# Berkeley-Speech-Group/sylber

Hardware: AMD Instinct MI355X
Metric: audio-sec/s encoded (sylber_base, 16 kHz, batched 10 s clips) (higher is better)
Workload: dtype bf16

## Files before the change

### include/sylber_hip_dev.h

```cpp
#ifndef SYLBER_HIP_DEV_H
#define SYLBER_HIP_DEV_H
#include <stdint.h>
#include "sylber_hip.h"
#ifdef __cplusplus
extern "C" {
#endif
int sylber_debug_gemm_bench(int32_t M, int32_t N, int32_t K, int32_t ldx, int32_t epi, int32_t act, int32_t cfg,
                            int32_t iters, float* ms_out);
int sylber_debug_gemm_pick(int32_t M, int32_t N, int32_t K, int32_t epi, int32_t act, int32_t fmt, int32_t model, int32_t kpat);
int sylber_debug_gemm_trace(int32_t M, int32_t N, int32_t K, int32_t ldx, int32_t epi, int32_t act, unsigned long long* out20,
                            float* ms_out);
int sylber_debug_poison_workspace(sylber_t h, int32_t byte);
int sylber_debug_conv0_scale_shift(sylber_t h, int32_t B, float* out_host);
int sylber_debug_attention_bench(int32_t B, int32_t T, int32_t precision, int32_t iters, float* ms_out);
#ifdef __cplusplus
}
#endif
#endif
```

### sylber_amd/_lib.py

```python
from __future__ import annotations

import ctypes
import os
from ctypes import POINTER, c_char_p, c_float, c_int, c_int32, c_int64, c_void_p

_HERE = os.path.dirname(os.path.abspath(__file__))
LIB_PATH = os.path.join(_HERE, "libsylber_hip.so")
_DEV_LIB = False
MAX_LAYERS = 12

c_float_p = POINTER(c_float)


class SylberLayerWeights(ctypes.Structure):
    _fields_ = [(n, c_float_p) for n in (
        "q_w", "q_b", "k_w", "k_b", "v_w", "v_b", "o_w", "o_b", "ln1_w", "ln1_b",
        "ff1_w", "ff1_b", "ff2_w", "ff2_b", "ln2_w", "ln2_b")]


class SylberMlpHidden(ctypes.Structure):
    _fields_ = [(n, c_float_p) for n in ("lin_w", "lin_b", "ff1_w", "ff1_b", "ff2_w", "ff2_b", "ln_w", "ln_b")]


class SylberMlpWeights(ctypes.Structure):
# ... 154 lines not shown
    "sylber_forward_packed": (c_int, [c_void_p, c_void_p, POINTER(c_int32), c_int32, c_void_p, c_void_p]),
    "sylber_packed_gather": (c_int, [c_void_p, POINTER(c_int32), c_int32, c_void_p, c_void_p]),
    "sylber_segment_packed": (c_int, [c_void_p, c_void_p, POINTER(c_int32), c_int32, c_float, c_float, c_void_p, c_void_p, c_void_p,
                                      c_void_p]),
    "sylber_cfm_packed_layout": (c_int, [POINTER(c_int32), c_int32, POINTER(c_int32)]),
    "sylber_cfm_workspace_bytes_packed": (c_int64, [c_void_p, POINTER(c_int32), c_int32]),
    "sylber_cfm_sample_packed": (c_int, [c_void_p, c_void_p, POINTER(c_int32), c_int32, c_int32, c_void_p, c_float, c_void_p, c_void_p,
                                         c_void_p]),
    "sylber_condition_packed_workspace_floats": (c_int64, [c_void_p, c_int32, c_int32]),
    "sylber_condition_packed": (c_int, [c_void_p, c_void_p, POINTER(c_int32), POINTER(c_int32), c_int32, c_void_p, c_void_p, c_void_p,
                                        c_int32, c_int32, c_float, c_void_p, c_void_p, c_void_p, c_void_p]),
    "sylber_condition_units_packed": (c_int, [c_void_p, c_void_p, c_int32, c_void_p, c_int32, c_void_p, c_void_p, c_void_p,
                                              POINTER(c_int32), c_int32, c_int32, c_void_p, c_void_p, c_void_p]),
    "sylber_op_attention": (c_int, [c_void_p, c_void_p, c_void_p, c_void_p, c_void_p, c_int32, c_int32, c_int32,
                                    c_int32, c_void_p]),
}
DEV_EXPORTS = {
    "sylber_debug_gemm_bench": (c_int, [c_int32] * 8 + [POINTER(c_float)]),
    "sylber_debug_gemm_pick": (c_int, [c_int32] * 8),
    "sylber_debug_gemm_trace": (c_int, [c_int32] * 6 + [POINTER(ctypes.c_uint64), POINTER(c_float)]),
    "sylber_debug_attention_bench": (c_int, [c_int32] * 4 + [POINTER(c_float)]),
    "sylber_debug_poison_workspace": (c_int, [c_void_p, c_int32]),
    "sylber_debug_conv0_scale_shift": (c_int, [c_void_p, c_int32, c_void_p]),
}
OPT_GEMM_TILE, OPT_ATTN_QUERIES_PER_WAVE, OPT_GEMM_PERSISTENT = 1, 2, 3
OPT_FUSE_OUTPROJ_LN, OPT_CONV0_VALU = 4, 5
OPT_FP8_ATTENTION, OPT_SEGMENT, OPT_PER_UTTERANCE = 7, 9, 14
TAP_CONV0, TAP_PROJ, TAP_POSCONV = -1, -2, -3
LTAP_QKV, LTAP_CTX, LTAP_ATTN_SUM, LTAP_LN1, LTAP_FFN1, LTAP_FFN2_SUM = 0, 1, 2, 3, 4, 5
LTAP_WIDTH = {LTAP_QKV: 2304, LTAP_CTX: 768, LTAP_ATTN_SUM: 768, LTAP_LN1: 768, LTAP_FFN1: 3072, LTAP_FFN2_SUM: 768}


def TAP_LAYER(l: int, k: int) -> int:
    return -(8 * (int(l) + 1) + int(k))


_LIB = None


class SylberHipError(RuntimeError):
    pass


def load() -> ctypes.CDLL:
    global _LIB
    if _LIB is None:
# ... 26 lines not shown
```

### sylber_amd/csrc/api.hip

```cpp
#include "ctx.h"

static thread_local char g_err[512] = "";
void syl_set_error(const char* what, const char* detail) { snprintf(g_err, sizeof(g_err), "%s: %s", what, detail); }
extern "C" const char* sylber_last_error(void) { return g_err; }

struct Packer {
    std::vector<char> host;
    size_t add(size_t bytes) { size_t off = (host.size() + 255) & ~(size_t)255; host.resize(off + bytes); return off; }
    size_t add_f32(const float* src, size_t n) { size_t o = add(n * 4); memcpy(host.data() + o, src, n * 4); return o; }
    int fmt = FMT_BF16;
    size_t add_bf16(const float* src, size_t n) {
        if (fmt == FMT_SPLIT) {
            size_t o = add(n * 4);
            bf16_t* d = (bf16_t*)(host.data() + o);
            for (size_t i = 0; i < n; ++i) { d[i] = f2h_host(src[i]); d[n + i] = f2h_host(src[i] - h2f_host(d[i])); }
            return o;
        }
        size_t o = add(n * 2);
        bf16_t* d = (bf16_t*)(host.data() + o);
        if (fmt == FMT_F16) for (size_t i = 0; i < n; ++i) d[i] = f2h_host(src[i]);
        else for (size_t i = 0; i < n; ++i) d[i] = f2bf(src[i]);
        return o;
    }
};
// ... 14 lines not shown
    size_t o_gnw = P.add_f32(w->gn_w, 512), o_gnb = P.add_f32(w->gn_b, 512);
    size_t o_conv[7] = {0};
    for (int i = 1; i < 7; ++i) {
        const int k = CK[i];
        const bool chunk_major = k == 3 && !f32 && c->fmt_conv != FMT_SPLIT;
        std::vector<float> tmp((size_t)512 * k * 512);
        for (int o = 0; o < 512; ++o)
            for (int cc = 0; cc < 512; ++cc)
                for (int j = 0; j < k; ++j) tmp[((size_t)o * k + j) * 512 + cc] = w->conv_w[i][((size_t)o * 512 + cc) * k + j];
        if (chunk_major) {
            std::vector<float> t2(tmp.size());
            for (int o = 0; o < 512; ++o)
                for (int pos = 0; pos < 1536; ++pos)
                    t2[(size_t)o * 1536 + pos] = tmp[(size_t)o * 1536 + tap3_offset(pos * 2) / 2];
            tmp.swap(t2);
        }
        o_conv[i] = f32 ? P.add_f32(tmp.data(), tmp.size()) : P.add_bf16(tmp.data(), tmp.size());
    }
    P.fmt = c->fmt;
    size_t o_fplw = P.add_f32(w->fp_ln_w, 512), o_fplb = P.add_f32(w->fp_ln_b, 512);
    size_t o_fpw = f32 ? P.add_f32(w->fp_w, 768 * 512) : P.add_bf16(w->fp_w, 768 * 512), o_fpb = P.add_f32(w->fp_b, 768);
    size_t o_posw;
    {
        std::vector<float> tmp((size_t)16 * 128 * 64 * 56, 0.f);
        for (int g = 0; g < 16; ++g)
            for (int n = 0; n < 48; ++n)
                for (int cc = 0; cc < 48; ++cc)
                    for (int t = 0; t < 128; ++t)
                        tmp[(((size_t)g * 128 + t) * 64 + n) * 56 + cc] = w->pos_w[(((size_t)g * 48 + n) * 48 + cc) * 128 + t];
        if (!f32) o_posw = P.add_bf16(tmp.data(), tmp.size());
        else {
            std::vector<float> t32((size_t)16 * 128 * 64 * 52, 0.f);
            for (int g = 0; g < 16; ++g)
                for (int n = 0; n < 48; ++n)
                    for (int cc = 0; cc < 48; ++cc)
                        for (int t = 0; t < 128; ++t)
                            t32[(((size_t)g * 128 + t) * 64 + n) * 52 + cc] = w->pos_w[(((size_t)g * 48 + n) * 48 + cc) * 128 + t];
            o_posw = P.add_f32(t32.data(), t32.size());
        }
    }
    size_t o_posb = P.add_f32(w->pos_b, 768);
    size_t o_elw = P.add_f32(w->enc_ln_w, 768), o_elb = P.add_f32(w->enc_ln_b, 768);
    struct LOff { size_t wqkv, bqkv, wo, bo, l1w, l1b, w1, b1, w2, b2, l2w, l2b; } lo[SYLBER_MAX_LAYERS];
    for (int l = 0; l < w->num_layers; ++l) {
        const SylberLayerWeights& lw = w->layers[l];
        std::vector<float> qkv((size_t)2304 * 768), bq(2304);
        memcpy(qkv.data(), lw.q_w, 768 * 768 * 4);
        memcpy(qkv.data() + 768 * 768, lw.k_w, 768 * 768 * 4);
        memcpy(qkv.data() + 2 * 768 * 768, lw.v_w, 768 * 768 * 4);
        memcpy(bq.data(), lw.q_b, 768 * 4); memcpy(bq.data() + 768, lw.k_b, 768 * 4); memcpy(bq.data() + 1536, lw.v_b, 768 * 4);
        lo[l].wqkv = f32 ? P.add_f32(qkv.data(), qkv.size()) : P.add_bf16(qkv.data(), qkv.size()); lo[l].bqkv = P.add_f32(bq.data(), 2304);
        lo[l].wo = f32 ? P.add_f32(lw.o_w, 768 * 768) : P.add_bf16(lw.o_w, 768 * 768); lo[l].bo = P.add_f32(lw.o_b, 768);
        lo[l].l1w = P.add_f32(lw.ln1_w, 768); lo[l].l1b = P.add_f32(lw.ln1_b, 768);
        lo[l].w1 = f32 ? P.add_f32(lw.ff1_w, (size_t)3072 * 768) : P.add_bf16(lw.ff1_w, (size_t)3072 * 768); lo[l].b1 = P.add_f32(lw.ff1_b, 3072);
// ... 232 lines not shown
```

### sylber_amd/csrc/common.h

```cpp
#pragma once
#include <hip/hip_runtime.h>
#include <stdint.h>

typedef unsigned short bf16_t;
typedef __bf16 bf16x8_t __attribute__((ext_vector_type(8)));
typedef float f32x16_t __attribute__((ext_vector_type(16)));
typedef float f32x4_t __attribute__((ext_vector_type(4)));
typedef unsigned short u16x8_t __attribute__((ext_vector_type(8)));
typedef unsigned short u16x4_t __attribute__((ext_vector_type(4)));

#define SYL_HIDDEN 768
#define SYL_CONV 512
#define SYL_SLOT_SAMPLES 320
#define SYL_HEADS 12
#define SYL_HDIM 64
#define SYL_FFN 3072
#define SYL_POSK 128
#define SYL_POSG 16
#define SYL_POSC 48

__host__ __device__ __forceinline__ bf16_t f2bf(float f) {
    union { float f; uint32_t u; } v; v.f = f;
    uint32_t u = v.u;
    if ((u & 0x7fffffffu) > 0x7f800000u) return (bf16_t)((u >> 16) | 0x40);
    u += 0x7fffu + ((u >> 16) & 1u);
    return (bf16_t)(u >> 16);
}
__host__ __device__ __forceinline__ float bf2f(bf16_t h) {
    union { float f; uint32_t u; } v; v.u = ((uint32_t)h) << 16;
    return v.f;
}
typedef __bf16 bf16x2_t __attribute__((ext_vector_type(2)));
__device__ __forceinline__ uint32_t pack_bf16x2(float lo, float hi) {
    typedef float f32pair_t __attribute__((ext_vector_type(2)));
    const f32pair_t v = {lo, hi};
    return __builtin_bit_cast(uint32_t, __builtin_convertvector(v, bf16x2_t));
}
__device__ __forceinline__ bf16_t f2bf_dev(float f) { return __builtin_bit_cast(unsigned short, (__bf16)f); }

enum { FMT_BF16 = 0, FMT_F16 = 1, FMT_SPLIT = 2 };
typedef _Float16 f16x8_t __attribute__((ext_vector_type(8)));
typedef _Float16 f16x2_t __attribute__((ext_vector_type(2)));
#define SYL_Q_SCALE 0.18033688011112042f
template <int FMT> struct H16 {
    static __device__ __forceinline__ uint32_t pack2(float lo, float hi) { return pack_bf16x2(lo, hi); }
    static __device__ __forceinline__ uint32_t pack2_bounded(float lo, float hi) { return pack_bf16x2(lo, hi); }
    static __device__ __forceinline__ bf16_t cvt(float f) { return f2bf_dev(f); }
    static __device__ __forceinline__ float up(bf16_t h) { return bf2f(h); }
    static __device__ __forceinline__ f32x16_t mfma(bf16x8_t a, bf16x8_t b, f32x16_t c) {
        return __builtin_amdgcn_mfma_f32_32x32x16_bf16(a, b, c, 0, 0, 0);
    }
};
template <> struct H16<FMT_F16> {
    static __device__ __forceinline__ float sat(float f) { return __builtin_amdgcn_fmed3f(f, -65504.0f, 65504.0f); }
    static __device__ __forceinline__ uint32_t pack2(float lo, float hi) {
        typedef float f32pair_t __attribute__((ext_vector_type(2)));
        const f32pair_t v = {sat(lo), sat(hi)};
        return __builtin_bit_cast(uint32_t, __builtin_convertvector(v, f16x2_t));
    }
    static __device__ __forceinline__ uint32_t pack2_bounded(float lo, float hi) {
        typedef float f32pair_t __attribute__((ext_vector_type(2)));
        const f32pair_t v = {lo, hi};
        return __builtin_bit_cast(uint32_t, __builtin_convertvector(v, f16x2_t));
    }
    static __device__ __forceinline__ bf16_t cvt(float f) { return __builtin_bit_cast(unsigned short, (_Float16)sat(f)); }
    static __device__ __forceinline__ float up(bf16_t h) { return (float)__builtin_bit_cast(_Float16, h); }
    static __device__ __forceinline__ f32x16_t mfma(bf16x8_t a, bf16x8_t b, f32x16_t c) {
        return __builtin_amdgcn_mfma_f32_32x32x16_f16(__builtin_bit_cast(f16x8_t, a), __builtin_bit_cast(f16x8_t, b), c, 0, 0, 0);
    }
};
template <> struct H16<FMT_SPLIT> : H16<FMT_F16> {
    static __device__ __forceinline__ uint32_t pack2_lo(float lo, float hi, uint32_t hi2) {
        const f16x2_t h = __builtin_bit_cast(f16x2_t, hi2);
        return H16<FMT_F16>::pack2_bounded(lo - (float)h[0], hi - (float)h[1]);
    }
    static __device__ __forceinline__ bf16_t cvt_lo(float f, bf16_t hi) { return H16<FMT_F16>::cvt(f - H16<FMT_F16>::up(hi)); }
};
__host__ __forceinline__ bf16_t f2h_host(float f) {
    union { float f; uint32_t u; } v; v.f = f;
    const uint32_t sign = (v.u >> 16) & 0x8000u;
    uint32_t a = v.u & 0x7fffffffu;
    if (a > 0x7f800000u) return (bf16_t)(sign | 0x7e00u);
    if (a >= 0x477ff000u) return (bf16_t)(sign | 0x7bffu);
    if (a < 0x38800000u) {
        if (a < 0x33000000u) return (bf16_t)sign;
        const int e = (int)(a >> 23);
        const uint32_t m = (a & 0x7fffffu) | 0x800000u;
        const int shift = 126 - e;
        uint32_t r = m >> shift;
        const uint32_t rem = m & ((1u << shift) - 1u), half = 1u << (shift - 1);
        if (rem > half || (rem == half && (r & 1u))) ++r;
// ... 133 lines not shown
```

### sylber_amd/csrc/forward.hip

```cpp
#include "ctx.h"

extern "C" int32_t sylber_num_frames(int32_t n) {
    for (int i = 0; i < 7; ++i) n = (n - CK[i]) / CS[i] + 1;
    return n;
}

static int frames_needed(int Lmax) {
    int n = Lmax, tp = 0;
    for (int i = 0; i < 7; ++i) {
        n = (n - CK[i]) / CS[i] + 1;
        const int f = 1 << (6 - i);
        const int need = (n + f - 1) / f;
        tp = need > tp ? need : tp;
    }
    return tp;
}
static int padded_frames(int Lmax) { return (frames_needed(Lmax) + 31) & ~31; }
extern "C" int32_t sylber_padded_frames(int32_t n_samples) { return n_samples < 400 ? 0 : padded_frames(n_samples); }

#define SYL_SLOT_ALIGN 64
extern "C" int sylber_packed_layout(const int32_t* samples_host, int32_t B, int32_t* offsets, int32_t* frames) {
    if (!samples_host || !offsets || !frames || B < 1) { syl_set_error("sylber_packed_layout", "need B >= 1 and non-null arrays"); return 1; }
    const long long cap = (long long)INT32_MAX / SYL_SLOT_SAMPLES;
    long long off = 0;
// ... 315 lines not shown
        return g;
    }
    void residual(GemmArgs& g, const float* gamma, const float* beta) const {
        g.out0 = w.pre; g.ld0 = 768; g.res = w.pre; g.ldres = 768; g.ln_stats = w.stats; g.ln_gamma = gamma; g.ln_beta = beta;
    }

    int projection() {
        LnArgs a = {};
        a.in = feats; a.in_bf16 = 1; a.ld_in = 512; a.gamma = c->fp_ln_w; a.beta = c->fp_ln_b;
        a.out_bf16 = w.ln512; a.ld_bf16 = 512; a.M = M; a.D = 512; a.fmt = c->fmt; a.fmt_in = c->fmt_conv;
        a.in_lo = feats_lo; a.out_lo = p.lo_ln512;
        RUN("ln512", launch_layernorm(a, s));
        GemmArgs g = linear(w.ln512, p.lo_ln512, c->fp_w, c->fp_b, 768, 512);
        g.out0 = w.xf32; g.ld0 = 768; g.out1 = w.xpad; g.Tp = p.Tp; g.T = p.T; g.valid = w.valid; g.xpad_rows = p.Tp + 128; g.out_lo = p.lo_xpad;
        RUN("gemm_proj", launch_gemm_bf16(EPI_PROJ, g, s));
        if (pk) RUN("zero_slot_tails", launch_zero_slot_tails(w.xf32, w.xpad, pk->slot, pk->frames, pk->nclip, pk->tail_max, s));
        AUDIT(aud_e, AUD_LN512, w.ln512, M, 512, 512);
        AUDIT(aud_e, AUD_XPAD, w.xpad, (long)B * (p.Tp + 128), 768, 768);
        return 0;
    }

    int posconv() {
        if (pk) RUN("posconv", launch_posconv_packed(w.xpad, c->pos_w, c->pos_b, w.xf32, w.pre, pk->nclip, pk->slot_max, pk->slot, pk->frames, s, c->fmt));
        else RUN("posconv", launch_posconv(w.xpad, c->pos_w, c->pos_b, w.xf32, w.pre, B, p.Tp, split ? 2 : 1, s, c->fmt, p.lo_xpad, (long)16 * 128 * 64 * 56));
        return 0;
    }

    int layernorm(const float* gam, const float* bet, bool last) {
        LnArgs a = {};
        a.in = w.pre; a.in_bf16 = 0; a.ld_in = 768; a.gamma = gam; a.beta = bet; a.M = M; a.D = 768; a.fmt = c->fmt; a.fmt_in = c->fmt;
        if (last) { a.out_f32 = hidden_dev; a.ld_f32 = 768; a.Tp = p.Tp; a.T = p.T; }
        else if (f8) { a.out_fp8 = w8.h; a.ld_fp8 = 768; a.out_scale = w8.hs; a.scale_rows = w8.Mp; a.out_stats = w.stats; }
        else { a.out_bf16 = w.h; a.ld_bf16 = 768; a.out_stats = w.stats; a.out_lo = p.lo_hbf; }
        if (launch_layernorm(a, s)) return 1;
        AUDIT(aud_e && !last && !f8, AUD_LN, w.h, M, 768, 768);
        return 0;
    }

    int tap_rows16(const bf16_t* buf, long lo, int W) {
        tapped = true;
        RUN("copy_out", launch_bf16_to_f32_rows(buf, W, hidden_dev, B, p.Tp, p.T, W, s, c->fmt, lo));
        return 0;
    }
    int tap_pre() { tapped = true; return copy_frames_f32(w.pre, hidden_dev, B, p.Tp, p.T, s); }

    int layer16(const LayerDev& d, bool last, int tk) {
        GemmArgs g = linear(w.h, p.lo_hbf, d.wqkv, d.bqkv, 2304, 768);
// ... 333 lines not shown
```

### sylber_amd/csrc/frontend.hip

```cpp
#include <stdlib.h>

#include "kernels.h"

#define NSTAT 65
#define C0_ROWS 256

__global__ __launch_bounds__(256) void conv0_stats_kernel(const float* __restrict__ wav, int Lmax, int L0, int chunk,
                                                          double* __restrict__ partials, int nchunk, const int* __restrict__ rows,
                                                          const int* __restrict__ slot) {
    const int b = blockIdx.y, ck = blockIdx.x;
    const float* x = wav + (slot ? (size_t)SYL_SLOT_SAMPLES * slot[b] : (size_t)b * Lmax);
    if (rows) {
        L0 = rows[b];
        const int nck = (L0 + 2047) / 2048;
        chunk = (L0 + nck - 1) / nck;
    }
    const int l0 = ck * chunk;
    const int l1 = min(L0, l0 + chunk);
    double acc[NSTAT];
#pragma unroll
    for (int i = 0; i < NSTAT; ++i) acc[i] = 0.0;
    for (int l = l0 + threadIdx.x; l < l1; l += 256) {
        float v[10];
#pragma unroll
// ... 181 lines not shown
    const int l_blk = bx * C0_ROWS;
    __syncthreads();
    for (int i = tid; i < C0_ROWS * 5 + 16; i += 256) {
        const int idx = 5 * l_blk + i;
        xs[i] = idx < Lmax ? x[idx] : 0.f;
    }
    __syncthreads();
#pragma unroll 1
    for (int rb = 0; rb < 2; ++rb) {
        const int lrow0 = wave * 64 + rb * 32;
        const int l0 = l_blk + lrow0;
        if (l0 >= R0) break;
        f16x8_t xh, xl;
        {
            const float* xr = xs + 5 * (lrow0 + ml) + 8 * h;
#pragma unroll
            for (int j = 0; j < 8; ++j) {
                const float v = xr[j];
                const _Float16 vh = (_Float16)v;
                xh[j] = vh; xl[j] = (_Float16)(v - (float)vh);
            }
        }
        const bool live = l0 + ml < L0;
#pragma unroll 1
        for (int q4 = 0; q4 < 4; ++q4) {
#pragma unroll
            for (int bi = 0; bi < 4; ++bi) {
                const int blk = q4 * 4 + bi;
                const f16x8_t whi = *(const f16x8_t*)(wfr + (blk * 64 + lane) * 32);
                const f16x8_t wlo = *(const f16x8_t*)(wfr + (blk * 64 + lane) * 32 + 16);
                f32x16_t acc;
#pragma unroll
                for (int g = 0; g < 4; ++g) {
                    const float4 sv = *(const float4*)(shf + 32 * blk + 8 * g + 4 * h);
                    acc[4 * g + 0] = sv.x; acc[4 * g + 1] = sv.y; acc[4 * g + 2] = sv.z; acc[4 * g + 3] = sv.w;
                }
                acc = __builtin_amdgcn_mfma_f32_32x32x16_f16(whi, xh, acc, 0, 0, 0);
                acc = __builtin_amdgcn_mfma_f32_32x32x16_f16(whi, xl, acc, 0, 0, 0);
                acc = __builtin_amdgcn_mfma_f32_32x32x16_f16(wlo, xh, acc, 0, 0, 0);
#pragma unroll
                for (int g = 0; g < 4; ++g) {
                    float y0 = gelu_fast(acc[4 * g + 0]), y1 = gelu_fast(acc[4 * g + 1]), y2 = gelu_fast(acc[4 * g + 2]), y3 = gelu_fast(acc[4 * g + 3]);
                    if (!live) { y0 = y1 = y2 = y3 = 0.f; }
                    uint2 pk; pk.x = H16<FMT>::pack2(y0, y1); pk.y = H16<FMT>::pack2(y2, y3);
                    *(uint2*)(stg + ml * (256 + 16) + (32 * bi + 8 * g + 4 * h) * 2) = pk;
                }
            }
#pragma unroll
            for (int it = 0; it < 8; ++it) {
                const int idx = it * 64 + lane;
                const int r = idx >> 4, ch = idx & 15;
                typedef unsigned int u32x4_t __attribute__((ext_vector_type(4)));
                const u32x4_t v = *(const u32x4_t*)(stg + r * (256 + 16) + ch * 16);
                const int l = l0 + r;
                if constexpr (NOSTORE) { if (v.x == 0x7fc1dead && l < 0) out[0] = (bf16_t)v.y; }
                else if (l < R0) __builtin_nontemporal_store(v, (u32x4_t*)(out + (obase + l) * SYL_CONV + q4 * 128 + ch * 8));
            }
        }
    }
    }
}

int launch_conv0_stats(const float* wav, int B, int Lmax, int L0, double* partials, int nchunk, hipStream_t s, const int* rows, const int* slot) {
    const int chunk = (L0 + nchunk - 1) / nchunk;
    hipLaunchKernelGGL(conv0_stats_kernel, dim3(nchunk, B), dim3(256), 0, s, wav, Lmax, L0, chunk, partials, nchunk, rows, slot);
    HIP_TRY(hipGetLastError());
    return 0;
}
int launch_conv0_finalize(const double* partials, int nchunk, const float* w0, const float* gn_w, const float* gn_b, int B,
                          int L0, float* scale_shift, hipStream_t s, const int* rows) {
    hipLaunchKernelGGL(conv0_finalize_kernel, dim3(B), dim3(512), 0, s, partials, nchunk, w0, gn_w, gn_b, L0, scale_shift, rows);
    HIP_TRY(hipGetLastError());
    return 0;
}
int launch_conv0_gn_gelu(const float* wav, int B, int Lmax, int L0, int R0, const float* w0, const float* scale_shift,
                         void* out, int out_f32, hipStream_t s, int fmt, long out_lo, int valu16) {
    dim3 grid((R0 + C0_ROWS - 1) / C0_ROWS, B);
    if (out_f32)
        hipLaunchKernelGGL((conv0_gn_gelu_kernel<true, true, FMT_BF16>), grid, dim3(256), 0, s, wav, Lmax, L0, R0, w0, scale_shift, out, 0L);
    else if (fmt == FMT_SPLIT)
        hipLaunchKernelGGL((conv0_gn_gelu_kernel<false, true, FMT_SPLIT>), grid, dim3(256), 0, s, wav, Lmax, L0, R0, w0, scale_shift, out, out_lo);
// ... 230 lines not shown
```

### sylber_amd/csrc/kernels.h

```cpp
#pragma once
#include "common.h"

enum GemmAct { ACT_NONE = 0, ACT_GELU_FAST = 1, ACT_GELU_ERF = 2, ACT_GELU_ERF7 = 3 };
enum GemmEpi {
    EPI_BF16 = 0,
    EPI_F32 = 1,
    EPI_F32_RES = 2,
    EPI_QK = 3,
    EPI_PROJ = 4,
    EPI_MXFP8 = 7,
    EPI_QK8 = 8,
    EPI_F32_RESLN = 6,
};

struct GemmArgs {
    const bf16_t* X; long ldx;
    const bf16_t* W;
    int M, N, K;
    int M_store;
    const float* bias;
    int act;
    void* out0; long ld0;
    void* out1; void* out2;
    const float* res; long ldres;
// ... 82 lines not shown
    const float* gamma; const float* beta;
    float* out_f32; long ld_f32;
    bf16_t* out_bf16; long ld_bf16;
    uint8_t* out_fp8; long ld_fp8;
    uint8_t* out_scale; long scale_rows;
    float* out_stats;
    int M, D;
    int Tp, T;
    long in_lo, out_lo;
};
int launch_layernorm(const LnArgs& a, hipStream_t s);

int launch_attention(const bf16_t* q, const bf16_t* k, const bf16_t* vt, const int* valid, bf16_t* ctx, int B, int T,
                     int Tp, int Tpv, int qw, hipStream_t s, int fmt = 0, long lo_qk = 0, long lo_vt = 0, long lo_ctx = 0);
int launch_attention_f8(const uint8_t* q8, const uint8_t* qs, const uint8_t* k8, const uint8_t* ks, const uint8_t* v8, const uint8_t* vs,
                        const int* valid, void* ctx, uint8_t* ctx_scale, long scale_rows, int B, int T, int Tp, int Tpv, hipStream_t s);
int launch_attention_f8out(const bf16_t* q, const bf16_t* k, const bf16_t* vt, const int* valid, uint8_t* ctx8, uint8_t* ctx_scale,
                           long scale_rows, int B, int T, int Tp, int Tpv, int qw, hipStream_t s);
int launch_attention_f32(const float* q, const float* k, const float* v, const int* valid, float* ctx, int B, int T,
                         int Tp, hipStream_t s);

int launch_posconv(const bf16_t* xpad, const bf16_t* wpk, const float* bias, const float* x_f32, float* out, int B,
                   int Tp, int act, hipStream_t s, int fmt = 0, long x_lo = 0, long w_lo = 0);
int launch_posconv_f32(const float* xpad, const float* w, const float* bias, const float* x_f32, float* out, int B,
                       int Tp, hipStream_t s);

int launch_segment(const float* hidden, int B, int T, int D, float norm_thr, float merge_thr, int64_t* seg, int* nseg,
                   float* feat, float* scratch, hipStream_t s, int mode = 0, const int* frames = nullptr, const int* row0 = nullptr);
size_t segment_scratch_floats(int B, int T, int D);

int launch_upload_ints(int* dst, const int32_t* vals_host, int n, int add, hipStream_t s);
int launch_f32_to_bf16(const float* in, bf16_t* out, size_t n, hipStream_t s);
int launch_f32_to_split16(const float* in, bf16_t* out, long lo_off, size_t n, hipStream_t s);
int launch_bf16_to_f32_rows(const bf16_t* in, long ld_in, float* out, int B, int Tp, int T, int D, hipStream_t s, int fmt = 0, long in_lo = 0);
int launch_tap_qkv(const bf16_t* q, const bf16_t* k, const bf16_t* vt, float* out, int B, int T, int Tp, int Tpv, hipStream_t s, int fmt, long lo_qk, long lo_vt);
```

### sylber_amd/csrc/ops.hip

```cpp
#include "ctx.h"

struct TmpBuf {
    void* p = nullptr;
    ~TmpBuf() { if (p) hipFree(p); }
    int alloc(size_t bytes) { return hipMalloc(&p, bytes) == hipSuccess ? 0 : 1; }
};

static void decode_tile(int tile, GemmArgs& g) {
    if (tile >= 1000000) { g.tune_mfma16 = -1; tile -= 1000000; if (tile == 999) tile = -1; }
    const int t = tile >= 100000 ? tile / 100000 : 0;
    if (tile >= 100000) tile %= 100000;
    g.tune_tail = t == 0 ? 0 : (t == 1 ? -1 : t - 1);
    g.tune_cfg = tile < 0 ? 0 : tile % 1000 + 1;
    g.tune_persist = tile >= 9000 ? -1 : (tile >= 1000 ? tile / 1000 : 0);
}

extern "C" int sylber_op_linear(const float* a_dev, const float* w_dev, const float* bias_dev, float* c_dev, int32_t M,
                                int32_t N, int32_t K, int32_t act, int32_t precision, int32_t tile, void* stream) {
    hipStream_t s = (hipStream_t)stream;
    if (precision == SYLBER_FP8) {
        if (K % 128 != 0) { syl_set_error("sylber_op_linear", "fp8 needs K % 128 == 0"); return 1; }
        TmpBuf a8, as, w8, wsc;
        const long Mp = ((long)M + 255) & ~255L, Np = ((long)N + 255) & ~255L;
        if (a8.alloc((size_t)M * K) || as.alloc((size_t)Mp * (K / 32)) || w8.alloc((size_t)N * K) || wsc.alloc((size_t)Np * (K / 32))) {
// ... 228 lines not shown
    const int qw = queries_per_wave == 32 ? 1 : (queries_per_wave == 64 ? 2 : 0);
    TmpBuf qb, kb, vb, cb;
    const size_t n = (size_t)B * Tp * 768;
    if (qb.alloc(n * 2) || kb.alloc(n * 2 + 64 * 64 * 2) || vb.alloc((size_t)B * 768 * Tpv * 2) || cb.alloc(n * 2)) { syl_set_error("sylber_op_attention", "alloc"); return 1; }
    HIP_TRY(hipMemsetAsync(qb.p, 0, n * 2, s)); HIP_TRY(hipMemsetAsync(kb.p, 0, n * 2 + 64 * 64 * 2, s));
    HIP_TRY(hipMemsetAsync(vb.p, 0, (size_t)B * 768 * Tpv * 2, s)); HIP_TRY(hipMemsetAsync(cb.p, 0, n * 2, s));
    hipLaunchKernelGGL(pack_qkv_kernel, dim3(T, B), dim3(256), 0, s, q_dev, k_dev, v_dev, (bf16_t*)qb.p, (bf16_t*)kb.p, (bf16_t*)vb.p, T, Tp, Tpv);
    if (launch_attention((bf16_t*)qb.p, (bf16_t*)kb.p, (bf16_t*)vb.p, valid_dev, (bf16_t*)cb.p, B, T, Tp, Tpv, qw, s)) return 1;
    if (launch_bf16_to_f32_rows((bf16_t*)cb.p, 768, o_dev, B, Tp, T, 768, s)) return 1;
    HIP_TRY(hipStreamSynchronize(s));
    return 0;
}


__global__ void fill_random_bf16(bf16_t* p, size_t n, unsigned seed);
extern "C" int sylber_debug_poison_workspace(sylber_t c, int32_t byte) {
    if (!c) { syl_set_error("sylber_debug_poison_workspace", "null handle"); return 1; }
    GUARD_DEVICE(c->device);
    HIP_TRY(hipDeviceSynchronize());
    if (c->ws) HIP_TRY(hipMemset(c->ws, byte & 0xff, c->ws_bytes));
    if (c->seg_scratch) HIP_TRY(hipMemset(c->seg_scratch, byte & 0xff, c->seg_scratch_floats * 4));
    c->ws_B = 0; c->ws_Lmax = 0;
    graphs_clear(c);
    return 0;
}

extern "C" int sylber_debug_conv0_scale_shift(sylber_t c, int32_t B, float* out_host) {
    if (!c || !out_host) { syl_set_error("sylber_debug_conv0_scale_shift", "null argument"); return 1; }
    if (!c->dbg_ss || !c->ws || B < 1 || B != c->dbg_ss_B) { syl_set_error("sylber_debug_conv0_scale_shift", "B must be the batch size of the handle's last forward"); return 1; }
    GUARD_DEVICE(c->device);
    HIP_TRY(hipDeviceSynchronize());
    HIP_TRY(hipMemcpy(out_host, c->dbg_ss, (size_t)B * SYL_CONV * 2 * sizeof(float), hipMemcpyDeviceToHost));
    return 0;
}

extern "C" int sylber_debug_attention_bench(int32_t B, int32_t T, int32_t precision, int32_t iters, float* ms_out) {
    const int Tp = (T + 31) & ~31, Tpv = (Tp + 63) & ~63;
    const size_t n = (size_t)B * Tp * 768;
    TmpBuf qin;
    if (qin.alloc((size_t)B * T * 768 * 4 * 3)) { syl_set_error("sylber_debug_attention_bench", "alloc"); return 1; }
    float* q = (float*)qin.p; float* k = q + (size_t)B * T * 768; float* v = k + (size_t)B * T * 768;
    const bool zero_data = iters < 0;
    if (zero_data) { iters = -iters; HIP_TRY(hipMemset(qin.p, 0, (size_t)B * T * 768 * 4 * 3)); }
    else
    {
        TmpBuf tmp;
// ... 195 lines not shown
```

### sylber_amd/csrc/posconv.hip

```cpp
#include "kernels.h"

#define PC_BM 256
#define PC_XROW 112
#define PC_XWIN (384 * PC_XROW)
#define PC_SLAB (64 * 112)
#define PC_TAPS_PER_STEP 2
#define PC_STEP (PC_TAPS_PER_STEP * PC_SLAB)
#define PC_LDS (PC_XWIN + 2 * PC_STEP)

typedef __attribute__((address_space(3))) void* lds_vptr;
typedef const __attribute__((address_space(1))) void* glb_vptr;
__device__ __forceinline__ void glds16p(__amdgpu_buffer_rsrc_t rs, int voff, int soff, void* l) {
    __builtin_amdgcn_raw_ptr_buffer_load_lds(rs, (lds_vptr)l, 16, voff, soff, 0, 0);
}

template <int ACT, int FMT>
__global__ __launch_bounds__(512, 4) void posconv_bf16_kernel(const bf16_t* __restrict__ xpad, const bf16_t* __restrict__ wpk,
                                                              const float* __restrict__ bias, const float* __restrict__ x_f32,
                                                              float* __restrict__ out, int Tp, long x_lo, long w_lo,
                                                              const int* __restrict__ slot, const int* __restrict__ frames) {
    extern __shared__ __attribute__((aligned(256))) char smem[];
    char* xwin = smem;
    char* wring = smem + PC_XWIN;
    const int tid = threadIdx.x, wave = tid >> 6, lane = tid & 63;
    const int ql = lane & 31, h = lane >> 5;
    const int t0 = blockIdx.x * PC_BM, g = blockIdx.y, b = blockIdx.z;
    const int rows_per_b = Tp + 128;
    int s0 = 0, Tb = 0, Tpb = Tp;
    if (slot) {
        s0 = slot[b]; Tb = frames[b]; Tpb = slot[b + 1] - s0;
        if (t0 >= Tpb) return;
    }

    f32x16_t acc[2];
#pragma unroll
    for (int i = 0; i < 2; ++i)
#pragma unroll
        for (int r = 0; r < 16; ++r) acc[i][r] = 0.f;
    constexpr int NPASS = FMT == FMT_SPLIT ? 3 : 1;
#pragma unroll 1
    for (int pass = 0; pass < NPASS; ++pass) {
    if (pass > 0) __syncthreads();
    {
        const bf16_t* xb = xpad + (pass == 1 ? x_lo : 0L) + (slot ? (size_t)s0 : (size_t)b * rows_per_b) * SYL_HIDDEN + g * SYL_POSC;
#pragma unroll
        for (int i = 0; i < 5; ++i) {
            const int idx = tid + 512 * i;
            if (idx < 384 * 6) {
                const int r = idx / 6, ch = idx - r * 6;
                uint4 v;
                if (slot) {
                    const int f = t0 + r - 64;
                    v = (f >= 0 && f < Tb) ? *(const uint4*)(xb + (size_t)(f + 64) * SYL_HIDDEN + ch * 8) : make_uint4(0u, 0u, 0u, 0u);
                } else {
                    int row = t0 + r; row = row < rows_per_b ? row : rows_per_b - 1;
                    v = *(const uint4*)(xb + (size_t)row * SYL_HIDDEN + ch * 8);
                }
                *(uint4*)(xwin + r * PC_XROW + ch * 16) = v;
            }
        }
    }
    const char* wg_base = (const char*)(wpk + (pass == 2 ? w_lo : 0L)) + (size_t)g * SYL_POSK * PC_SLAB;
    const __amdgpu_buffer_rsrc_t rwg = __builtin_amdgcn_make_buffer_rsrc((void*)wg_base, 0, (int)0xffffffffu, 0x00020000);
    auto stage = [&](int step, int buf) {
        char* dst = wring + buf * PC_STEP;
#pragma unroll
        for (int i = 0; i < 2; ++i) {
            const int piece = wave + 8 * i;
            if (piece < 14) glds16p(rwg, piece * 1024 + lane * 16, step * PC_STEP, dst + piece * 1024);
        }
    };

    const int xfrag = (wave * 32 + ql) * PC_XROW + h * 16;
    const int wfrag = ql * 112 + h * 16;
    const int nsteps = SYL_POSK / PC_TAPS_PER_STEP;
    stage(0, 0);
    for (int st = 0; st < nsteps; ++st) {
        asm volatile("s_waitcnt vmcnt(0)" ::: "memory");
        __syncthreads();
        if (st + 1 < nsteps) stage(st + 1, (st + 1) & 1);
        const char* wb = wring + (st & 1) * PC_STEP;
#pragma unroll
        for (int tt = 0; tt < PC_TAPS_PER_STEP; ++tt) {
            const int tap = st * PC_TAPS_PER_STEP + tt;
#pragma unroll
            for (int q = 0; q < 3; ++q) {
                const bf16x8_t xf = *(const bf16x8_t*)(xwin + xfrag + tap * PC_XROW + q * 32);
#pragma unroll
                for (int nf = 0; nf < 2; ++nf) {
                    const bf16x8_t wf = *(const bf16x8_t*)(wb + tt * PC_SLAB + nf * 32 * 112 + wfrag + q * 32);
                    acc[nf] = H16<FMT>::mfma(wf, xf, acc[nf]);
                }
            }
        }
    }
    }
    const int t = t0 + wave * 32 + ql;
    if (t < Tpb) {
        const size_t m = slot ? (size_t)s0 + t : (size_t)b * Tp + t;
#pragma unroll
        for (int nf = 0; nf < 2; ++nf)
#pragma unroll
            for (int gg = 0; gg < 4; ++gg) {
                const int nl = 32 * nf + 8 * gg + 4 * h;
                if (nl >= SYL_POSC) continue;
                const int n = g * SYL_POSC + nl;
                const float4 bb = *(const float4*)(bias + n);
                const float4 rr = *(const float4*)(x_f32 + m * SYL_HIDDEN + n);
                float v0 = acc[nf][4 * gg + 0] + bb.x, v1 = acc[nf][4 * gg + 1] + bb.y;
                float v2 = acc[nf][4 * gg + 2] + bb.z, v3 = acc[nf][4 * gg + 3] + bb.w;
                if constexpr (ACT == 2 && FMT == FMT_SPLIT) { v0 = gelu_erf7(v0); v1 = gelu_erf7(v1); v2 = gelu_erf7(v2); v3 = gelu_erf7(v3); }
                else if constexpr (ACT == 2) { v0 = gelu_erf(v0); v1 = gelu_erf(v1); v2 = gelu_erf(v2); v3 = gelu_erf(v3); }
                else { v0 = gelu_fast(v0); v1 = gelu_fast(v1); v2 = gelu_fast(v2); v3 = gelu_fast(v3); }
                *(float4*)(out + m * SYL_HIDDEN + n) = make_float4(rr.x + v0, rr.y + v1, rr.z + v2, rr.w + v3);
            }
    }
}

static int posconv_attrs() {
    static PerDeviceOnce attr_once;
    if (attr_once.need()) {
        HIP_TRY(hipFuncSetAttribute((const void*)posconv_bf16_kernel<1, FMT_BF16>, hipFuncAttributeMaxDynamicSharedMemorySize, PC_LDS));
        HIP_TRY(hipFuncSetAttribute((const void*)posconv_bf16_kernel<2, FMT_BF16>, hipFuncAttributeMaxDynamicSharedMemorySize, PC_LDS));
        HIP_TRY(hipFuncSetAttribute((const void*)posconv_bf16_kernel<1, FMT_F16>, hipFuncAttributeMaxDynamicSharedMemorySize, PC_LDS));
        HIP_TRY(hipFuncSetAttribute((const void*)posconv_bf16_kernel<2, FMT_SPLIT>, hipFuncAttributeMaxDynamicSharedMemorySize, PC_LDS));
    }
    return 0;
}

int launch_posconv(const bf16_t* xpad, const bf16_t* wpk, const float* bias, const float* x_f32, float* out, int B, int Tp,
                   int act, hipStream_t s, int fmt, long x_lo, long w_lo) {
    dim3 grid((Tp + PC_BM - 1) / PC_BM, SYL_POSG, B);
    if (posconv_attrs()) return 1;
    if (fmt == FMT_SPLIT) {
        hipLaunchKernelGGL((posconv_bf16_kernel<2, FMT_SPLIT>), grid, dim3(512), PC_LDS, s, xpad, wpk, bias, x_f32, out, Tp, x_lo, w_lo, nullptr, nullptr);
        HIP_TRY(hipGetLastError());
        return 0;
    }
    if (fmt == FMT_F16 && act == 2) { syl_set_error("launch_posconv", "the erf GELU (act 2) has no fp16 instantiation"); return 1; }
// ... 18 lines not shown
```

Measured before the change: 68530.

## Rework positional conv to 16x16x32 MFMA with dense swizzled weight packing

Result: no change. 68740, median of 6 (+0.3%).

```diff
diff --git a/include/sylber_hip_dev.h b/include/sylber_hip_dev.h
--- a/include/sylber_hip_dev.h
+++ b/include/sylber_hip_dev.h
@@ -12,6 +12,7 @@
                             float* ms_out);
 int sylber_debug_poison_workspace(sylber_t h, int32_t byte);
 int sylber_debug_conv0_scale_shift(sylber_t h, int32_t B, float* out_host);
+int sylber_debug_posconv_pack(const float* pos_w, int32_t precision, uint16_t* out_host);
 int sylber_debug_attention_bench(int32_t B, int32_t T, int32_t precision, int32_t iters, float* ms_out);
 #ifdef __cplusplus
 }
diff --git a/sylber_amd/_lib.py b/sylber_amd/_lib.py
--- a/sylber_amd/_lib.py
+++ b/sylber_amd/_lib.py
@@ -200,6 +200,7 @@
     "sylber_debug_attention_bench": (c_int, [c_int32] * 4 + [POINTER(c_float)]),
     "sylber_debug_poison_workspace": (c_int, [c_void_p, c_int32]),
     "sylber_debug_conv0_scale_shift": (c_int, [c_void_p, c_int32, c_void_p]),
+    "sylber_debug_posconv_pack": (c_int, [c_void_p, c_int32, c_void_p]),
 }
 OPT_GEMM_TILE, OPT_ATTN_QUERIES_PER_WAVE, OPT_GEMM_PERSISTENT = 1, 2, 3
 OPT_FUSE_OUTPROJ_LN, OPT_CONV0_VALU = 4, 5
diff --git a/sylber_amd/csrc/api.hip b/sylber_amd/csrc/api.hip
--- a/sylber_amd/csrc/api.hip
+++ b/sylber_amd/csrc/api.hip
@@ -60,14 +60,11 @@
     size_t o_fpw = f32 ? P.add_f32(w->fp_w, 768 * 512) : P.add_bf16(w->fp_w, 768 * 512), o_fpb = P.add_f32(w->fp_b, 768);
     size_t o_posw;
     {
-        std::vector<float> tmp((size_t)16 * 128 * 64 * 56, 0.f);
-        for (int g = 0; g < 16; ++g)
-            for (int n = 0; n < 48; ++n)
-                for (int cc = 0; cc < 48; ++cc)
-                    for (int t = 0; t < 128; ++t)
-                        tmp[(((size_t)g * 128 + t) * 64 + n) * 56 + cc] = w->pos_w[(((size_t)g * 48 + n) * 48 + cc) * 128 + t];
-        if (!f32) o_posw = P.add_bf16(tmp.data(), tmp.size());
-        else {
+        if (!f32) {
+            std::vector<float> tmp((size_t)SYL_HIDDEN * SYL_POSC * SYL_POSK);
+            posconv_pack_host(w->pos_w, tmp.data());
+            o_posw = P.add_bf16(tmp.data(), tmp.size());
+        } else {
             std::vector<float> t32((size_t)16 * 128 * 64 * 52, 0.f);
             for (int g = 0; g < 16; ++g)
                 for (int n = 0; n < 48; ++n)
diff --git a/sylber_amd/csrc/common.h b/sylber_amd/csrc/common.h
--- a/sylber_amd/csrc/common.h
+++ b/sylber_amd/csrc/common.h
@@ -18,6 +18,10 @@
 #define SYL_POSK 128
 #define SYL_POSG 16
 #define SYL_POSC 48
+#define SYL_POSW_K 96
+__host__ __device__ __forceinline__ int posconv_kgroup_tap(int kgi) { return kgi >= 6 ? 1 : 0; }
+__host__ __device__ __forceinline__ int posconv_kgroup_octet(int kgi) { return kgi >= 6 ? kgi - 6 : kgi; }
+__host__ __device__ __forceinline__ int posconv_wswz(int n) { return (0x78 >> (((n >> 2) & 3) * 2)) & 3; }
 
 __host__ __device__ __forceinline__ bf16_t f2bf(float f) {
     union { float f; uint32_t u; } v; v.f = f;
@@ -50,6 +54,9 @@
     static __device__ __forceinline__ f32x16_t mfma(bf16x8_t a, bf16x8_t b, f32x16_t c) {
         return __builtin_amdgcn_mfma_f32_32x32x16_bf16(a, b, c, 0, 0, 0);
     }
+    static __device__ __forceinline__ f32x4_t mfma16(bf16x8_t a, bf16x8_t b, f32x4_t c) {
+        return __builtin_amdgcn_mfma_f32_16x16x32_bf16(a, b, c, 0, 0, 0);
+    }
 };
 template <> struct H16<FMT_F16> {
     static __device__ __forceinline__ float sat(float f) { return __builtin_amdgcn_fmed3f(f, -65504.0f, 65504.0f); }
@@ -67,6 +74,9 @@
     static __device__ __forceinline__ float up(bf16_t h) { return (float)__builtin_bit_cast(_Float16, h); }
     static __device__ __forceinline__ f32x16_t mfma(bf16x8_t a, bf16x8_t b, f32x16_t c) {
         return __builtin_amdgcn_mfma_f32_32x32x16_f16(__builtin_bit_cast(f16x8_t, a), __builtin_bit_cast(f16x8_t, b), c, 0, 0, 0);
+    }
+    static __device__ __forceinline__ f32x4_t mfma16(bf16x8_t a, bf16x8_t b, f32x4_t c) {
+        return __builtin_amdgcn_mfma_f32_16x16x32_f16(__builtin_bit_cast(f16x8_t, a), __builtin_bit_cast(f16x8_t, b), c, 0, 0, 0);
     }
 };
 template <> struct H16<FMT_SPLIT> : H16<FMT_F16> {
diff --git a/sylber_amd/csrc/forward.hip b/sylber_amd/csrc/forward.hip
--- a/sylber_amd/csrc/forward.hip
+++ b/sylber_amd/csrc/forward.hip
@@ -361,7 +361,7 @@
 
     int posconv() {
         if (pk) RUN("posconv", launch_posconv_packed(w.xpad, c->pos_w, c->pos_b, w.xf32, w.pre, pk->nclip, pk->slot_max, pk->slot, pk->frames, s, c->fmt));
-        else RUN("posconv", launch_posconv(w.xpad, c->pos_w, c->pos_b, w.xf32, w.pre, B, p.Tp, split ? 2 : 1, s, c->fmt, p.lo_xpad, (long)16 * 128 * 64 * 56));
+        else RUN("posconv", launch_posconv(w.xpad, c->pos_w, c->pos_b, w.xf32, w.pre, B, p.Tp, split ? 2 : 1, s, c->fmt, p.lo_xpad, (long)SYL_HIDDEN * SYL_POSC * SYL_POSK));
         return 0;
     }
 
diff --git a/sylber_amd/csrc/frontend.hip b/sylber_amd/csrc/frontend.hip
--- a/sylber_amd/csrc/frontend.hip
+++ b/sylber_amd/csrc/frontend.hip
@@ -1,4 +1,6 @@
 #include <stdlib.h>
+
+#include <type_traits>
 
 #include "kernels.h"
 
@@ -227,6 +229,7 @@
             }
         }
         const bool live = l0 + ml < L0;
+        auto rows32 = [&](auto all_live) {
 #pragma unroll 1
         for (int q4 = 0; q4 < 4; ++q4) {
 #pragma unroll
@@ -246,7 +249,7 @@
 #pragma unroll
                 for (int g = 0; g < 4; ++g) {
                     float y0 = gelu_fast(acc[4 * g + 0]), y1 = gelu_fast(acc[4 * g + 1]), y2 = gelu_fast(acc[4 * g + 2]), y3 = gelu_fast(acc[4 * g + 3]);
-                    if (!live) { y0 = y1 = y2 = y3 = 0.f; }
+                    if constexpr (!decltype(all_live)::value) { if (!live) { y0 = y1 = y2 = y3 = 0.f; } }
                     uint2 pk; pk.x = H16<FMT>::pack2(y0, y1); pk.y = H16<FMT>::pack2(y2, y3);
                     *(uint2*)(stg + ml * (256 + 16) + (32 * bi + 8 * g + 4 * h) * 2) = pk;
                 }
@@ -262,6 +265,9 @@
                 else if (l < R0) __builtin_nontemporal_store(v, (u32x4_t*)(out + (obase + l) * SYL_CONV + q4 * 128 + ch * 8));
             }
         }
+        };
+        if (__builtin_amdgcn_readfirstlane(l0) + 32 <= L0) rows32(std::true_type{});
+        else rows32(std::false_type{});
     }
     }
 }
diff --git a/sylber_amd/csrc/kernels.h b/sylber_amd/csrc/kernels.h
--- a/sylber_amd/csrc/kernels.h
+++ b/sylber_amd/csrc/kernels.h
@@ -128,6 +128,7 @@
 
 int launch_posconv(const bf16_t* xpad, const bf16_t* wpk, const float* bias, const float* x_f32, float* out, int B,
                    int Tp, int act, hipStream_t s, int fmt = 0, long x_lo = 0, long w_lo = 0);
+void posconv_pack_host(const float* pos_w, float* out);
 int launch_posconv_f32(const float* xpad, const float* w, const float* bias, const float* x_f32, float* out, int B,
                        int Tp, hipStream_t s);
 
diff --git a/sylber_amd/csrc/ops.hip b/sylber_amd/csrc/ops.hip
--- a/sylber_amd/csrc/ops.hip
+++ b/sylber_amd/csrc/ops.hip
@@ -274,6 +274,20 @@
     if (c->seg_scratch) HIP_TRY(hipMemset(c->seg_scratch, byte & 0xff, c->seg_scratch_floats * 4));
     c->ws_B = 0; c->ws_Lmax = 0;
     graphs_clear(c);
+    return 0;
+}
+
+extern "C" int sylber_debug_posconv_pack(const float* pos_w, int32_t precision, uint16_t* out_host) {
+    if (!pos_w || !out_host) { syl_set_error("sylber_debug_posconv_pack", "null argument"); return 1; }
+    if (precision != SYLBER_BF16 && precision != SYLBER_FP16 && precision != SYLBER_SPLIT16) { syl_set_error("sylber_debug_posconv_pack", "bf16, fp16 or split16"); return 1; }
+    const size_t n = (size_t)SYL_HIDDEN * SYL_POSC * SYL_POSK;
+    std::vector<float> tmp(n);
+    posconv_pack_host(pos_w, tmp.data());
+    for (size_t i = 0; i < n; ++i) {
+        if (precision == SYLBER_BF16) out_host[i] = f2bf(tmp[i]);
+        else out_host[i] = f2h_host(tmp[i]);
+        if (precision == SYLBER_SPLIT16) out_host[n + i] = f2h_host(tmp[i] - h2f_host(out_host[i]));
+    }
     return 0;
 }
 
diff --git a/sylber_amd/csrc/posconv.hip b/sylber_amd/csrc/posconv.hip
--- a/sylber_amd/csrc/posconv.hip
+++ b/sylber_amd/csrc/posconv.hip
@@ -1,11 +1,11 @@
 #include "kernels.h"
 
 #define PC_BM 256
-#define PC_XROW 112
+#define PC_XROW 128
 #define PC_XWIN (384 * PC_XROW)
-#define PC_SLAB (64 * 112)
+#define PC_WROW (SYL_POSW_K * 2)
 #define PC_TAPS_PER_STEP 2
-#define PC_STEP (PC_TAPS_PER_STEP * PC_SLAB)
+#define PC_STEP (SYL_POSC * PC_WROW)
 #define PC_LDS (PC_XWIN + 2 * PC_STEP)
 
 typedef __attribute__((address_space(3))) void* lds_vptr;
@@ -23,7 +23,7 @@
     char* xwin = smem;
     char* wring = smem + PC_XWIN;
     const int tid = threadIdx.x, wave = tid >> 6, lane = tid & 63;
-    const int ql = lane & 31, h = lane >> 5;
+    const int fl = lane & 15, kg = lane >> 4;
     const int t0 = blockIdx.x * PC_BM, g = blockIdx.y, b = blockIdx.z;
     const int rows_per_b = Tp + 128;
     int s0 = 0, Tb = 0, Tpb = Tp;
@@ -32,11 +32,20 @@
         if (t0 >= Tpb) return;
     }
 
-    f32x16_t acc[2];
+    f32x4_t acc[3][2];
 #pragma unroll
-    for (int i = 0; i < 2; ++i)
+    for (int i = 0; i < 3; ++i)
 #pragma unroll
-        for (int r = 0; r < 16; ++r) acc[i][r] = 0.f;
+        for (int j = 0; j < 2; ++j) acc[i][j] = f32x4_t{0.f, 0.f, 0.f, 0.f};
+    int xrow[3], xoct[3], xph[3];
+#pragma unroll
+    for (int q = 0; q < 3; ++q) {
+        const int kgi = 4 * q + kg, tt = posconv_kgroup_tap(kgi), oc = posconv_kgroup_octet(kgi);
+        xrow[q] = (wave * 32 + fl + tt) * PC_XROW;
+        xoct[q] = oc * 16;
+        xph[q] = ((fl + tt) >> 1) * 32;
+    }
+    const int wfrag = fl * PC_WROW + ((kg ^ posconv_wswz(fl)) * 16);
     constexpr int NPASS = FMT == FMT_SPLIT ? 3 : 1;
 #pragma unroll 1
     for (int pass = 0; pass < NPASS; ++pass) {
@@ -56,65 +65,71 @@
                     int row = t0 + r; row = row < rows_per_b ? row : rows_per_b - 1;
                     v = *(const uint4*)(xb + (size_t)row * SYL_HIDDEN + ch * 8);
                 }
-                *(uint4*)(xwin + r * PC_XROW + ch * 16) = v;
+                *(uint4*)(xwin + r * PC_XROW + ((ch ^ (((r >> 1) & 3) << 1)) * 16)) = v;
             }
         }
     }
-    const char* wg_base = (const char*)(wpk + (pass == 2 ? w_lo : 0L)) + (size_t)g * SYL_POSK * PC_SLAB;
+    const char* wg_base = (const char*)(wpk + (pass == 2 ? w_lo : 0L)) + (size_t)g * (SYL_POSK / PC_TAPS_PER_STEP) * PC_STEP;
     const __amdgpu_buffer_rsrc_t rwg = __builtin_amdgcn_make_buffer_rsrc((void*)wg_base, 0, (int)0xffffffffu, 0x00020000);
     auto stage = [&](int step, int buf) {
         char* dst = wring + buf * PC_STEP;
-#pragma unroll
-        for (int i = 0; i < 2; ++i) {
-            const int piece = wave + 8 * i;
-            if (piece < 14) glds16p(rwg, piece * 1024 + lane * 16, step * PC_STEP, dst + piece * 1024);
-        }
+        glds16p(rwg, wave * 1024 + lane * 16, step * PC_STEP, dst + wave * 1024);
+        if (wave == 0) glds16p(rwg, 8 * 1024 + lane * 16, step * PC_STEP, dst + 8 * 1024);
     };
 
-    const int xfrag = (wave * 32 + ql) * PC_XROW + h * 16;
-    const int wfrag = ql * 112 + h * 16;
     const int nsteps = SYL_POSK / PC_TAPS_PER_STEP;
     stage(0, 0);
     for (int st = 0; st < nsteps; ++st) {
         asm volatile("s_waitcnt vmcnt(0)" ::: "memory");
         __syncthreads();
         if (st + 1 < nsteps) stage(st + 1, (st + 1) & 1);
-        const char* wb = wring + (st & 1) * PC_STEP;
+        const char* wb = wring + (st & 1) * PC_STEP + wfrag;
+        const char* xb = xwin + st * (PC_TAPS_PER_STEP * PC_XROW);
 #pragma unroll
-        for (int tt = 0; tt < PC_TAPS_PER_STEP; ++tt) {
-            const int tap = st * PC_TAPS_PER_STEP + tt;
+        for (int q = 0; q < 3; ++q) {
+            const char* xq = xb + xrow[q] + (xoct[q] ^ ((xph[q] + st * 32) & 96));
+            const bf16x8_t xf0 = *(const bf16x8_t*)xq;
+            const bf16x8_t xf1 = *(const bf16x8_t*)(xq + 16 * PC_XROW);
 #pragma unroll
-            for (int q = 0; q < 3; ++q) {
-                const bf16x8_t xf = *(const bf16x8_t*)(xwin + xfrag + tap * PC_XROW + q * 32);
-#pragma unroll
-                for (int nf = 0; nf < 2; ++nf) {
-                    const bf16x8_t wf = *(const bf16x8_t*)(wb + tt * PC_SLAB + nf * 32 * 112 + wfrag + q * 32);
-                    acc[nf] = H16<FMT>::mfma(wf, xf, acc[nf]);
-                }
+            for (int nb = 0; nb < 3; ++nb) {
+                const bf16x8_t wf = *(const bf16x8_t*)(wb + nb * 16 * PC_WROW + q * 64);
+                acc[nb][0] = H16<FMT>::mfma16(wf, xf0, acc[nb][0]);
+                acc[nb][1] = H16<FMT>::mfma16(wf, xf1, acc[nb][1]);
             }
         }
     }
     }
-    const int t = t0 + wave * 32 + ql;
-    if (t < Tpb) {
+#pragma unroll
+    for (int fb = 0; fb < 2; ++fb) {
+        const int t = t0 + wave * 32 + fb * 16 + fl;
+        if (t >= Tpb) continue;
         const size_t m = slot ? (size_t)s0 + t : (size_t)b * Tp + t;
 #pragma unroll
-        for (int nf = 0; nf < 2; ++nf)
-#pragma unroll
-            for (int gg = 0; gg < 4; ++gg) {
-                const int nl = 32 * nf + 8 * gg + 4 * h;
-                if (nl >= SYL_POSC) continue;
-                const int n = g * SYL_POSC + nl;
-                const float4 bb = *(const float4*)(bias + n);
-                const float4 rr = *(const float4*)(x_f32 + m * SYL_HIDDEN + n);
-                float v0 = acc[nf][4 * gg + 0] + bb.x, v1 = acc[nf][4 * gg + 1] + bb.y;
-                float v2 = acc[nf][4 * gg + 2] + bb.z, v3 = acc[nf][4 * gg + 3] + bb.w;
-                if constexpr (ACT == 2 && FMT == FMT_SPLIT) { v0 = gelu_erf7(v0); v1 = gelu_erf7(v1); v2 = gelu_erf7(v2); v3 = gelu_erf7(v3); }
-                else if constexpr (ACT == 2) { v0 = gelu_erf(v0); v1 = gelu_erf(v1); v2 = gelu_erf(v2); v3 = gelu_erf(v3); }
-                else { v0 = gelu_fast(v0); v1 = gelu_fast(v1); v2 = gelu_fast(v2); v3 = gelu_fast(v3); }
-                *(float4*)(out + m * SYL_HIDDEN + n) = make_float4(rr.x + v0, rr.y + v1, rr.z + v2, rr.w + v3);
+        for (int nb = 0; nb < 3; ++nb) {
+            const int n = g * SYL_POSC + 16 * nb + 4 * kg;
+            const float4 bb = *(const float4*)(bias + n);
+            const float4 rr = *(const float4*)(x_f32 + m * SYL_HIDDEN + n);
+            float v0 = acc[nb][fb][0] + bb.x, v1 = acc[nb][fb][1] + bb.y;
+            float v2 = acc[nb][fb][2] + bb.z, v3 = acc[nb][fb][3] + bb.w;
+            if constexpr (ACT == 2 && FMT == FMT_SPLIT) { v0 = gelu_erf7(v0); v1 = gelu_erf7(v1); v2 = gelu_erf7(v2); v3 = gelu_erf7(v3); }
+            else if constexpr (ACT == 2) { v0 = gelu_erf(v0); v1 = gelu_erf(v1); v2 = gelu_erf(v2); v3 = gelu_erf(v3); }
+            else { v0 = gelu_fast(v0); v1 = gelu_fast(v1); v2 = gelu_fast(v2); v3 = gelu_fast(v3); }
+            *(float4*)(out + m * SYL_HIDDEN + n) = make_float4(rr.x + v0, rr.y + v1, rr.z + v2, rr.w + v3);
+        }
+    }
+}
+
+void posconv_pack_host(const float* pos_w, float* out) {
+    for (int g = 0; g < SYL_POSG; ++g)
+        for (int st = 0; st < SYL_POSK / 2; ++st)
+            for (int n = 0; n < SYL_POSC; ++n) {
+                float* row = out + (((size_t)g * (SYL_POSK / 2) + st) * SYL_POSC + n) * SYL_POSW_K;
+                for (int kgi = 0; kgi < 12; ++kgi) {
+                    const int tap = 2 * st + posconv_kgroup_tap(kgi), oc = posconv_kgroup_octet(kgi);
+                    const int p = (kgi & ~3) | ((kgi & 3) ^ posconv_wswz(n));
+                    for (int j = 0; j < 8; ++j) row[8 * p + j] = pos_w[(((size_t)g * SYL_POSC + n) * SYL_POSC + 8 * oc + j) * SYL_POSK + tap];
+                }
             }
-    }
 }
 
 static int posconv_attrs() {
```
